# toverainc/willow-inference-server

Measured on AMD Instinct MI355X. Metric: realtime_multiple (audio_ms / infer_ms), Whisper large-v2 beam=5, 3.84 s clip, higher is better.
Workload: dtype f16; 1 GPU; whisper-large beam=5 clip=3sec (3840 ms) batch=1/GPU, PCM resident in HBM -> ids on host; parallelism=1 independent replicas (utterance sharding, no data-path collective)

## Files before the change

### include/wis_hip.h

```cpp
#ifndef WIS_HIP_H
#define WIS_HIP_H

#include <stddef.h>
#include <stdint.h>

#ifdef __cplusplus
extern "C" {
#endif

#define WIS_ABI_VERSION 1

#define WIS_OK             0
#define WIS_E_ARG         -1
#define WIS_E_FORMAT      -2
#define WIS_E_NOMEM       -3
#define WIS_E_CHECKSUM    -4
#define WIS_E_HIP         -5
#define WIS_E_STATE       -6
#define WIS_E_UNSUPPORTED -7

#define WIS_SAMPLE_RATE 16000
#define WIS_N_FFT       400
#define WIS_HOP         160
#define WIS_N_MELS      80
// ... 152 lines not shown
                          int B, int R, int H, int T, int chunks);
int wis_op_dec_cross_attn_folded(int device, const float* q_raw, const float* xres, const float* qcs, const float* qb,
                                 const void* kx_f16, const void* vt_f16, void* out_f16, int B, int R, int H, int T, int chunks);

int wis_op_dec_cross_attn_stat(int device, const float* q, const float* q2, const float* stat, const float* qcs, const float* qb,
                               const void* kx_f16, const void* vt_f16, void* out_f16, int B, int R, int H, int T, int chunks,
                               int out_mb, int kv_shared, int no_spin);
int wis_op_dec_self_attn_ex(int device, const float* q, const void* kc_f16, const void* vc_f16, const int32_t* pos, void* out_f16,
                            int M, int H, int ctx, int rpu, int sstride, int rmul, int nb, int out_mb,
                            const int32_t* anc, int w0, int aw, const int32_t* base);
int wis_op_gemv_qkv(int device, const float* x, const float* gamma, const float* beta, const void* W_f16, const float* bias,
                    const int32_t* slot, const int32_t* pos, float* q, void* kc_f16, void* vc_f16, int M, int d, int ctx);
int wis_op_gemv_out_cq(int device, const void* a_f16, const float* x0, const void* Wo_f16, const float* bo, const void* Wq_f16, const float* bq,
                       const float* gamma, const float* beta, float* x1, float* stat, float* q, float* q2, float* qcs, float* qb,
                       int M, int d, int force_frag);

typedef struct wis_sv wis_sv_t;
typedef struct {
  int32_t conv_dim;
  int32_t n_conv_layers;
  int32_t conv_kernel[8], conv_stride[8];
  int32_t hidden_size, n_heads, n_layers, intermediate_size;
  int32_t num_conv_pos_embeddings, num_conv_pos_embedding_groups;
  int32_t num_buckets, max_bucket_distance;
  int32_t n_tdnn;
  int32_t tdnn_dim[8], tdnn_kernel[8], tdnn_dilation[8];
  int32_t xvector_output_dim;
  int64_t max_samples;
} wis_sv_config_t;
int    wis_sv_create(const wis_sv_config_t* cfg, const void* arena, size_t arena_bytes, int arena_on_device,
// ... 21 lines not shown
```

### willow-inference-server_amd/csrc/dec_kernels.hip

```cpp
#include <string.h>
#include "common.hpp"
#include "kernels.hpp"

namespace wis {

__global__ void pack_gemv_kernel(const f16* __restrict__ W, f16* __restrict__ Wp, int N, int Npad, int K, int n_scale, float scale, int rows) {
  const int ksteps = K / 32;
  const size_t total = (size_t)Npad * ksteps * 4;
  for (size_t idx = (size_t)blockIdx.x * blockDim.x + threadIdx.x; idx < total; idx += (size_t)gridDim.x * blockDim.x) {
    const int row = (int)(idx % rows);
    size_t t = idx / rows;
    const int kq = (int)(t & 3); t >>= 2;
    const int ks = (int)(t % ksteps), nt = (int)(t / ksteps);
    const int n = rows * nt + row, k = 32 * ks + 8 * kq;
    f16x8 v;
    if (n < N) {
      v = *reinterpret_cast<const f16x8*>(W + (size_t)n * K + k);
      if (n < n_scale) {
#pragma unroll
        for (int j = 0; j < 8; ++j) v[j] = (f16)((float)v[j] * scale);
      }
    } else {
#pragma unroll
      for (int j = 0; j < 8; ++j) v[j] = (f16)0.f;
// ... 421 lines not shown
#define WIS_GV_LEAD_DECL(s) const void* s##x, const void* s##x2, const f16* s##Wp, int s##M, int s##N, int s##K, int s##xsplit
#define WIS_GV_LEAD_APPLY(q, s) (q).x = s##x; (q).x2 = s##x2; (q).Wp = s##Wp; (q).M = s##M; (q).N = s##N; (q).K = s##K; (q).xsplit = s##xsplit
template <int MB, int MODE, int SC, int RM, bool W8, int NT = 1>
__global__ __launch_bounds__(256) void gemv_kernel(WIS_GV_LEAD_DECL(l_), int KC, GemvP p) {
  extern __shared__ __attribute__((aligned(16))) char smem[];
  WIS_GV_LEAD_APPLY(p, l_);
  gemv_body<MB, MODE, SC, RM, W8, NT>(p, KC, blockIdx.x, smem);
}
template <int SCA, int SCB>
__global__ __launch_bounds__(256) void gemv_dual_kernel(int nA, int M, const void* ax, const f16* aWp, const void* bx, const void* bx2, const f16* bWp, int bxsplit,
                                                        GemvP pa, GemvP pb) {
  extern __shared__ __attribute__((aligned(16))) char smem[];
  if ((int)blockIdx.x < nA) { pa.x = ax; pa.x2 = nullptr; pa.Wp = aWp; pa.M = M; pa.K = SCA * 128; gemv_body<1, 2, SCA, 1, false>(pa, SCA * 128, blockIdx.x, smem); }
  else { pb.x = bx; pb.x2 = bx2; pb.Wp = bWp; pb.M = M; pb.K = SCB * 128; pb.xsplit = bxsplit; gemv_body<1, 2, SCB, 1, false>(pb, SCB * 128, (int)blockIdx.x - nA, smem); }
}
int launch_gemv_dual(hipStream_t st, const GemvP& pa, const GemvP& pb) {
  if (pa.M != pb.M || pa.M < 1 || pa.M > 16 || pa.x2 || pa.wscale || pb.wscale || (pa.flags & (GV_LN | GV_QKV)) || (pb.flags & (GV_LN | GV_QKV))) { set_error("gemv_dual: unsupported pair"); return WIS_E_UNSUPPORTED; }
  if (pa.M * (pa.K / 8) > 13 * 256 || pb.M * (pb.K / 8) > 13 * 256 || pa.K % 128 || pb.K % 128) { set_error("gemv_dual: rows do not fit the register staging (M=%d K=%d/%d)", pa.M, pa.K, pb.K); return WIS_E_UNSUPPORTED; }
  const int sa = pa.K / 128, sb = pb.K / 128;
  const size_t aux = (size_t)4 * 64 * 16 + MAX_ROWS * 8 + 4 * 16 * 4 + 16;
  const int Kmax = pa.K > pb.K ? pa.K : pb.K;
  const size_t lds = (((size_t)pa.M * (Kmax + 8) * 2 + 15) & ~(size_t)15) + aux;
  if (lds > 65536) { set_error("gemv_dual: LDS"); return WIS_E_UNSUPPORTED; }
  const int nA = cdiv(pa.N, 16), nB = cdiv(pb.N, 16);
  dim3 grid(nA + nB), block(256);
  GemvP a = pa, b = pb; a.rows = 16; b.rows = 16;
  if (sa == 10 && sb == 20) hipLaunchKernelGGL((gemv_dual_kernel<10, 20>), grid, block, lds, st, nA, a.M, a.x, a.Wp, b.x, b.x2, b.Wp, b.xsplit, a, b);
  else if (sa == 8 && sb == 16) hipLaunchKernelGGL((gemv_dual_kernel<8, 16>), grid, block, lds, st, nA, a.M, a.x, a.Wp, b.x, b.x2, b.Wp, b.xsplit, a, b);
  else if (sa == 6 && sb == 12) hipLaunchKernelGGL((gemv_dual_kernel<6, 12>), grid, block, lds, st, nA, a.M, a.x, a.Wp, b.x, b.x2, b.Wp, b.xsplit, a, b);
  else if (sa == 4 && sb == 8) hipLaunchKernelGGL((gemv_dual_kernel<4, 8>), grid, block, lds, st, nA, a.M, a.x, a.Wp, b.x, b.x2, b.Wp, b.xsplit, a, b);
  else if (sa == 3 && sb == 6) hipLaunchKernelGGL((gemv_dual_kernel<3, 6>), grid, block, lds, st, nA, a.M, a.x, a.Wp, b.x, b.x2, b.Wp, b.xsplit, a, b);
  else { set_error("gemv_dual: K=%d/%d not instantiated", pa.K, pb.K); return WIS_E_UNSUPPORTED; }
  return WIS_OK;
// ... 543 lines not shown
  const int m = blockIdx.x;
  const f16* e = emb + (size_t)tok[m] * d;
  const f16* pe = pos_emb + (size_t)pos[m] * d;
  for (int i = threadIdx.x; i < d; i += blockDim.x) {
    const float v = (float)e[i] + (float)pe[i];
    x[(size_t)m * d + i] = v;
    if (xh) xh[(size_t)m * d + i] = (f16)v;
  }
}
int launch_dec_embed(hipStream_t st, const f16* emb, const f16* pos_emb, const int* tok, const int* pos, float* x, int M, int d, f16* xh) {
  hipLaunchKernelGGL(dec_embed_kernel, dim3(M), dim3(256), 0, st, emb, pos_emb, tok, pos, x, xh, d);
  return WIS_OK;
}

template <bool TREE, int NB>
__global__ __launch_bounds__(64) void dec_self_attn_kernel(const float* __restrict__ q, const f16* __restrict__ kc, const f16* __restrict__ vc,
                                                           const int* __restrict__ pos, int d, int ctx, int rpu, int sstride, int rmul,
                                                           f16* __restrict__ out, unsigned long long* prof, int out_mb,
                                                           const int* __restrict__ anc, int w0, int aw, const int* __restrict__ base) {
  __shared__ float red[4][64];
  const int m = blockIdx.x, h = blockIdx.y, lane = threadIdx.x, pl = lane >> 3, c = lane & 7;
  unsigned long long* pf = (m == 0 && h == 0 && lane == 0) ? prof : nullptr;
  if (lane == 0) tl_begin(prof);
  stamp(pf, 0);
  const int ls = TREE ? (base ? base[m] : anc[(size_t)m * aw]) : (m / rpu) * sstride + (m % rpu) * rmul;
  const int len = pos[m] + 1;
  auto slot_of = [&](int p) -> int {
    if (!TREE) return ls;
    int t = p - w0; t = t < aw - 1 ? t : aw - 1;
    return t < 0 ? ls : anc[(size_t)m * aw + t];
  };
  const float4 q0 = *reinterpret_cast<const float4*>(q + (size_t)m * d + h * 64 + 8 * c);
  const float4 q1 = *reinterpret_cast<const float4*>(q + (size_t)m * d + h * 64 + 8 * c + 4);
  const float qv[8] = {q0.x, q0.y, q0.z, q0.w, q1.x, q1.y, q1.z, q1.w};
// ... 72 lines not shown
  } while (p0 < len);
  stamp(pf, 2);
#pragma unroll
  for (int j = 0; j < 8; ++j) acc[j] += dpp_f<0x128>(acc[j]);
  if ((lane & 8) == 0) {
#pragma unroll
    for (int j = 0; j < 8; ++j) red[lane >> 4][8 * c + j] = acc[j];
  }
  __syncthreads();
  stamp(pf, 3);
  const float o = (red[0][lane] + red[1][lane]) + (red[2][lane] + red[3][lane]);
  out[out_mb ? xf_index(m, h * 64 + lane, out_mb) : (size_t)m * d + h * 64 + lane] = (f16)(o / l_run);
  stamp(pf, 4);
  if (lane == 0) tl_end(prof);
}
int launch_dec_self_attn(hipStream_t st, const SelfAttnP& p) {
  if (p.ctx > 512 || p.ctx < 64) { set_error("dec_self_attn: ctx=%d outside [64, 512]", p.ctx); return WIS_E_UNSUPPORTED; }
#define WIS_SA(TREEv, NBv) hipLaunchKernelGGL((dec_self_attn_kernel<TREEv, NBv>), dim3(p.M, p.H), dim3(64), 0, st, p.q, p.kc, p.vc, p.pos, p.d, p.ctx, p.rpu, p.sstride, p.rmul, p.out, \
                                              p.prof, p.out_mb, p.anc, p.w0, p.aw, p.base)
  if (p.anc) {
    if (p.aw < 1) { set_error("dec_self_attn: ancestor table of width %d", p.aw); return WIS_E_ARG; }
    WIS_SA(true, 8);
  } else if (p.nb == 2) WIS_SA(false, 2);
  else if (p.nb == 4) WIS_SA(false, 4);
  else WIS_SA(false, 8);
#undef WIS_SA
  return WIS_OK;
}

__device__ __forceinline__ void st_sc1(float* p, float v) {
  __hip_atomic_store(reinterpret_cast<unsigned*>(p), __float_as_uint(v), __ATOMIC_RELAXED, __HIP_MEMORY_SCOPE_AGENT);
}
// ... 1246 lines not shown
```

### willow-inference-server_amd/csrc/kernels.hpp

```cpp
#pragma once
#include "common.hpp"

namespace wis {

struct GemmP {
  const f16* A; int64_t a_bs; int a_rs; int a_rpb;
  const f16* W;
  int M, N, K;
  int klen;
  int n_span = 0, n_period = 0, n_phase = 0;
};
static inline GemmP gemm_plain(const f16* A, int lda, const f16* W, int M, int N, int K) {
  GemmP p; p.A = A; p.a_bs = 0; p.a_rs = lda; p.a_rpb = 0x7fffffff; p.W = W; p.M = M; p.N = N; p.K = K; p.klen = 0; return p;
}
int launch_layernorm(hipStream_t st, const float* x, const float* gamma, const float* beta, f16* y, int M, int d);
int launch_gemm_generic(hipStream_t st, const GemmP& p, const float* bias, const float* resid, void* C, int flags);
int launch_gemm_splitk_resid(hipStream_t st, const GemmP& p, int splits, float* scratch, const float* bias, const float* resid, float* X,
                             const float* ln_gamma = nullptr, const float* ln_beta = nullptr, f16* Y = nullptr);
int launch_gemm_conv1(hipStream_t st, const GemmP& p, const float* bias, f16* C, int T);
int launch_gemm_conv2(hipStream_t st, const GemmP& p, const float* bias, const float* pos, float* X, int T);
int launch_gemm_qkv(hipStream_t st, const GemmP& p, const float* bias, f16* qk, f16* vt, int d, int T, int Tpad, int H);
int launch_gemm_crosskv(hipStream_t st, const GemmP& p, const float* bias, f16* kx, f16* vt, int d, int T, int Tpad, int H, int64_t kx_lstride, int64_t vt_lstride);
int launch_enc_attention(hipStream_t st, const f16* qk, const f16* vt, f16* out, int B, int T, int Tpad, int H, float* part = nullptr, unsigned* counters = nullptr,
                         size_t part_cap = 0);
// ... 26 lines not shown
  float* q; f16* kc; f16* vc; const int* slot; const int* pos; int d; int ctx;
  unsigned long long* prof;
  int rows;
  const void* x2; int xsplit;
  f16* y16;
  int xmb;
  const float* stat_in;
  float* stat_out;
  f16* y_xf;
  int ymb;
  int ksplit; float* kpart; unsigned* kcnt;
  int mb0, mbi;
  int wks, wk0;
};
int launch_gemv(hipStream_t st, const GemvP& p);
int launch_gemv_dual(hipStream_t st, const GemvP& pa, const GemvP& pb);
int launch_gemv_frag(hipStream_t st, const GemvP& p);
int launch_gemv_frag3(hipStream_t st, const GemvP* p, int n);
__host__ __device__ static inline size_t xf_index(int m, int k, int MB) {
  return ((size_t)((k >> 5) * MB + (m >> 4)) * 64 + (m & 15) + 16 * ((k >> 3) & 3)) * 8 + (k & 7);
}
int launch_xf_pack(hipStream_t st, const void* x, int x_f16, f16* xf, float* stat, int M, int K, int MB);
int launch_dec_embed_xf(hipStream_t st, const f16* emb, const f16* pos_emb, const int* tok, const int* pos, float* x, f16* xf, float* stat, int M, int d, int MB);
int launch_fold_ln(hipStream_t st, f16* W, const float* gamma, const float* beta, float* bias, float* csum, int N, int K, int n_scale, float qscale);
int launch_csum8(hipStream_t st, const f16* W, const float* scale, float* csum, int N, int K, int n_scale, float qscale);
int launch_pack_gemv8(hipStream_t st, const f16* W, unsigned char* Wp, float* scale, int N, int Npad, int K, int n_scale, float qscale);
int launch_pack_gemv(hipStream_t st, const f16* W, f16* Wp, int N, int Npad, int K, int n_scale, float scale, int rows = 16);
int gemv_rows_for(int N, int K);

int launch_dec_embed(hipStream_t st, const f16* emb, const f16* pos_emb, const int* tok, const int* pos, float* x, int M, int d, f16* xh = nullptr);
struct SelfAttnP {
  const float* q = nullptr; const f16* kc = nullptr; const f16* vc = nullptr; const int* pos = nullptr; f16* out = nullptr;
  int M = 0, H = 0, d = 0, ctx = 0, rpu = 0, sstride = 0, rmul = 0;
  unsigned long long* prof = nullptr; int out_mb = 0; const int* anc = nullptr; int w0 = 0, aw = 0;
  const int* base = nullptr;
  int nb = 8;
};
int launch_dec_self_attn(hipStream_t st, const SelfAttnP& p);
constexpr int CA_SPIN_MAX_BH = 192;
struct CrossAttnP {
  const float* q = nullptr; const f16* kx = nullptr; const f16* vt = nullptr; f16* out = nullptr; float* part = nullptr; unsigned* counters = nullptr;
  int B = 0, R = 0, H = 0, d = 0, T = 0, Tpad = 0, chunks = 0;
  unsigned long long* prof = nullptr; int out_mb = 0;
  const float* xres = nullptr; const float* qcs = nullptr; const float* qb = nullptr;
  unsigned long long* gran = nullptr; unsigned* epoch = nullptr;
  const float* q2 = nullptr; int xres_is_stat = 0;
  int kv_shared = 0;
};
int launch_dec_cross_attn(hipStream_t st, const CrossAttnP& p);

struct SampleCfg {
// ... 57 lines not shown
```

### willow-inference-server_amd/csrc/model.hip

```cpp
#include <math.h>
#include <stdlib.h>
#include <string.h>
#include <time.h>
#include <algorithm>
#include <array>
#include <atomic>
#include <chrono>
#include <map>
#include <mutex>
#include <memory>
#include <string>
#include <vector>

#include "common.hpp"
#include "kernels.hpp"

using namespace wis;

namespace wis {

__global__ void convert_kernel(const void* __restrict__ src, int src_f16, void* __restrict__ dst, int dst_f16,
                               int64_t rows, int64_t cols, int64_t dst_ld, int64_t n_scale, float scale) {
  const int64_t total = rows * cols;
  for (int64_t i = (int64_t)blockIdx.x * blockDim.x + threadIdx.x; i < total; i += (int64_t)gridDim.x * blockDim.x) {
// ... 143 lines not shown
  std::vector<DecLayerW> dec;
  f16 *emb, *dec_pos; float *dec_ln_g, *dec_ln_b;
  DecProj proj;
  float *bias_all, *bias_begin; int* d_lang_ids;
  int n_vocab_pad;
  int Tpad;
  f16 *img, *c1, *xn, *qk, *vt, *ao, *hbuf, *mem;
  float* x; float* skbuf; float* enc_part = nullptr; unsigned* enc_cnt = nullptr;
  std::vector<f16*> kx, vx;
  std::vector<f16*> kc, vc;
  f16 *kc_all = nullptr, *vc_all = nullptr; size_t kv_layer_stride = 0;
  f16 *kx_all = nullptr, *vx_all = nullptr, *w_ckv_all = nullptr; float* b_ckv_all = nullptr;
  size_t kx_lstride = 0, vx_lstride = 0;
  float *dx, *dq, *logits, *part; f16 *dao, *dh, *dln; unsigned* counters;
  float* dq2 = nullptr;
  int sa_nb = 8;
  float* gf_part = nullptr; unsigned* gf_cnt = nullptr; int gf_ksplit = 1;
  unsigned long long* ca_gran = nullptr; unsigned* ca_epoch = nullptr;
  bool spin_off = false;
  int handoff_retries = 0;
  bool spin_now = true;
  f16 *dxf = nullptr, *daoxf = nullptr, *dhxf = nullptr; float* dstat = nullptr;
  RowMeta rm; BeamState bs;
  RowMeta rm_win;
  float *st_max, *st_sum, *st_val; int* st_idx;
  int* ts_desc = nullptr;
  float* d_nsp = nullptr;
  int nsp_B = 0;
  float* d_in; int64_t* d_nsamp; float* d_probs;
  int* vstep = nullptr; int* pick_tok = nullptr; float* pick_lp = nullptr;
// ... 277 lines not shown
  WIS_RET(dalloc(m, &m->kc_all, m->kv_layer_stride * L));
  WIS_RET(dalloc(m, &m->vc_all, m->kv_layer_stride * L));
  m->kx_lstride = (size_t)Bm * H * 8 * T * 8; m->vx_lstride = (size_t)Bm * H * 64 * m->Tpad;
  WIS_RET(dalloc(m, &m->kx_all, m->kx_lstride * L));
  WIS_RET(dalloc(m, &m->vx_all, m->vx_lstride * L));
  WIS_HIP_CHECK(hipMemsetAsync(m->vx_all, 0, m->vx_lstride * L * 2, m->st));
  for (int l = 0; l < L; ++l) {
    m->kx[l] = m->kx_all + (size_t)l * m->kx_lstride;
    m->vx[l] = m->vx_all + (size_t)l * m->vx_lstride;
    m->kc[l] = m->kc_all + (size_t)l * slots * ctx * d;
    m->vc[l] = m->vc_all + (size_t)l * slots * ctx * d;
  }
  WIS_RET(dalloc(m, &m->dx, (size_t)MAX_ROWS * d));
  WIS_RET(dalloc(m, &m->dq, (size_t)MAX_ROWS * d));
  WIS_RET(dalloc(m, &m->dq2, (size_t)MAX_ROWS * d));
  WIS_RET(dalloc(m, &m->dao, (size_t)MAX_ROWS * d));
  WIS_RET(dalloc(m, &m->dh, (size_t)MAX_ROWS * 4 * d));
  WIS_RET(dalloc(m, &m->dln, (size_t)MAX_ROWS * d));
  WIS_RET(dalloc(m, &m->dxh, (size_t)MAX_ROWS * d));
  {
    const size_t blk = (size_t)(MAX_ROWS / 16) * 64 * 8;
    WIS_RET(dalloc(m, &m->dxf, (size_t)(d / 32) * blk)); WIS_RET(dalloc(m, &m->daoxf, (size_t)(d / 32) * blk)); WIS_RET(dalloc(m, &m->dhxf, (size_t)(4 * d / 32) * blk));
    WIS_RET(dalloc(m, &m->dstat, (size_t)MAX_ROWS * (d / 16) * 2));
    WIS_HIP_CHECK(hipMemsetAsync(m->dxf, 0, (size_t)(d / 32) * blk * 2, m->st)); WIS_HIP_CHECK(hipMemsetAsync(m->daoxf, 0, (size_t)(d / 32) * blk * 2, m->st));
    WIS_HIP_CHECK(hipMemsetAsync(m->dhxf, 0, (size_t)(4 * d / 32) * blk * 2, m->st));
  }
  WIS_RET(dalloc(m, &m->logits, (size_t)MAX_ROWS * m->n_vocab_pad));
  const int Bg = Bm > MAX_ROWS / 16 ? Bm : MAX_ROWS / 16;
  WIS_RET(dalloc(m, &m->part, (size_t)Bg * H * 16 * 16 * 66));
  WIS_RET(dalloc(m, &m->counters, (size_t)Bg * H));
// ... 176 lines not shown
}

struct TreeWin { const int* anc; int w0, aw; const int* base = nullptr; };
int align_capture_q(wis_model* m, int l, int M);

static GemvP gemv_small(const DecProj& p, const void* x, void* y, int M, int flags) {
  GemvP g; memset(&g, 0, sizeof(g));
  g.x = x; g.csum = p.csum; g.Wp = p.Wp; g.wscale = p.scale; g.bias = p.bias; g.y = y; g.M = M; g.N = p.N; g.K = p.K; g.flags = flags; g.rows = p.rows;
  return g;
}
static GemvP gemv_frag(const DecProj& p, const void* xf, int M, int flags) {
  GemvP g; memset(&g, 0, sizeof(g));
  g.x = xf; g.csum = p.csum; g.Wp = p.Wp; g.wscale = p.scale; g.bias = p.bias; g.M = M; g.N = p.N; g.K = p.K; g.flags = flags; g.xmb = cdiv(M, 16); g.rows = 16;
  return g;
}
static void out_cq_dual(const DecLayerW& w, const f16* a, const f16* xh, float* x1, float* stat, float* q, int M, GemvP* ga, GemvP* gb) {
  const int d = w.out.K;
  memset(ga, 0, sizeof(*ga));
  ga->x = a; ga->Wp = w.out.Wp; ga->bias = w.out.bias; ga->y = x1; ga->M = M; ga->N = d; ga->K = d; ga->flags = GV_RESID; ga->stat_out = stat;
  memset(gb, 0, sizeof(*gb));
  gb->x = xh; gb->x2 = a; gb->xsplit = d; gb->Wp = w.cqo.Wp; gb->bias = w.cqo.bias; gb->y = q; gb->M = M; gb->N = d; gb->K = w.cqo.K; gb->flags = GV_OUT_F32;
}
static void out_cq_frag3(const DecLayerW& w, const f16* af, const f16* xf, float* x1, float* stat, float* q, float* q2, int M, GemvP g3[3]) {
  const int d = w.out.K;
  g3[0] = gemv_frag(w.out, af, M, GV_RESID);
  g3[0].wscale = nullptr; g3[0].y = x1; g3[0].ymb = g3[0].xmb; g3[0].stat_out = stat;
  g3[1] = gemv_frag(w.cqo, xf, M, GV_OUT_F32);
  g3[1].K = d; g3[1].y = q; g3[1].wks = w.cqo.K / 32; g3[1].wk0 = 0;
  g3[2] = gemv_frag(w.cqo, af, M, GV_OUT_F32);
  g3[2].K = d; g3[2].bias = nullptr; g3[2].y = q2; g3[2].wks = w.cqo.K / 32; g3[2].wk0 = d / 32;
}

static int dec_forward_frag(wis_model* m, int M, int R, int B, bool want_logits, int sstride, int rmul, int chunks, const TreeWin* tw = nullptr) {
  const wis_config_t& c = m->cfg; hipStream_t st = m->st;
  const int d = c.d_model, H = c.n_heads, T = c.n_audio_ctx, ctx = c.n_text_ctx, MB = cdiv(M, 16);
  if (tw && (M % 16 != 0 || R != 16 || B != M / 16)) { set_error("dec_forward_frag: a tree window takes whole groups of 16 rows"); return WIS_E_ARG; }
// ... 77 lines not shown
  const int ln = ln16 ? GV_LN16 : GV_LN;
  auto ln_x = [&](const f16* x16) { return ln16 ? (const void*)x16 : (const void*)m->dx; };
  WIS_RET(launch_dec_embed(st, m->emb, m->dec_pos, m->rm.tok, m->rm.pos, m->dx, M, d, fold ? m->dxh : nullptr));
  SelfAttnP sa;
  sa.q = m->dq; sa.pos = m->rm.pos; sa.out = m->dao; sa.M = M; sa.H = H; sa.d = d; sa.ctx = ctx; sa.rpu = R; sa.sstride = sstride; sa.rmul = rmul; sa.nb = m->sa_nb;
  CrossAttnP ca;
  ca.q = m->dq; ca.out = m->dao; ca.part = m->part; ca.counters = m->counters; ca.B = B; ca.R = R; ca.H = H; ca.d = d; ca.T = T; ca.Tpad = m->Tpad; ca.chunks = chunks;
  ca.gran = m->spin_now ? m->ca_gran : nullptr; ca.epoch = m->ca_epoch;
  for (int l = 0; l < c.n_dec_layers; ++l) {
    const DecLayerW& w = m->dec[l];
    unsigned long long* pr = (m->prof_on && (l == 0 || m->prof_all)) ? m->d_prof + (size_t)l * 8 * 16 : nullptr;
    GemvP g = gemv_small(w.qkv, ln_x(m->dxh), nullptr, M, ln | GV_QKV);
    g.q = m->dq; g.kc = m->kc[l]; g.vc = m->vc[l]; g.slot = m->rm.slot; g.pos = m->rm.pos; g.d = d; g.ctx = ctx;
    g.prof = pr;
    WIS_RET(launch_gemv(st, g));
    sa.kc = m->kc[l]; sa.vc = m->vc[l]; sa.prof = pr ? pr + 16 : nullptr;
    WIS_RET(launch_dec_self_attn(st, sa));
    ca.kx = m->kx[l]; ca.vt = m->vx[l]; ca.prof = pr ? pr + 64 : nullptr;
    if (fold) {
      GemvP ga, gb;
      out_cq_dual(w, m->dao, m->dxh, m->dx, m->dstat, m->dq, M, &ga, &gb);
      ga.prof = pr ? pr + 32 : nullptr;
      WIS_RET(launch_gemv_dual(st, ga, gb));
      CrossAttnP cf = ca;
      cf.xres = m->dstat; cf.qcs = w.cq.csum; cf.qb = w.cq.bias; cf.xres_is_stat = 1;
      WIS_RET(launch_dec_cross_attn(st, cf));
    } else {
    g = gemv_small(w.out, m->dao, m->dx, M, GV_RESID);
    g.prof = pr ? pr + 32 : nullptr;
    WIS_RET(launch_gemv(st, g));
    g = gemv_small(w.cq, m->dx, m->dq, M, GV_LN | GV_OUT_F32);
    g.prof = pr ? pr + 48 : nullptr;
    WIS_RET(launch_gemv(st, g));
    WIS_RET(launch_dec_cross_attn(st, ca));
    }
    g = gemv_small(w.cout, m->dao, m->dx, M, GV_RESID);
    g.prof = pr ? pr + 80 : nullptr;
    if (ln16) g.y16 = m->dln;
// ... 323 lines not shown
```

### willow-inference-server_amd/csrc/taps.hip

```cpp
extern "C" {

int wis_debug_encode(wis_model_t* m, const float* input, int input_kind, int B, float* enc_out) {
  if (!m || !input || !enc_out) { set_error("wis_debug_encode: bad argument"); return WIS_E_ARG; }
  WIS_ENTER(m, "wis_debug_encode")
  WIS_HIP_CHECK(hipSetDevice(m->device));
  WIS_RET(check_batch(m, B, 1));
  WIS_RET(stage_input(m, input, input_kind, B));
  WIS_RET(run_encoder(m, B));
  const int64_t n = (int64_t)B * m->cfg.n_audio_ctx * m->cfg.d_model;
  hipLaunchKernelGGL(f16_to_f32_kernel, dim3(blocks_for(n)), dim3(256), 0, m->st, m->mem, m->x, n);
  WIS_HIP_CHECK(hipMemcpyAsync(enc_out, m->x, (size_t)n * 4, hipMemcpyDeviceToHost, m->st));
  WIS_HIP_CHECK(hipStreamSynchronize(m->st));
  return WIS_OK;
}

int wis_debug_logits(wis_model_t* m, const float* input, int input_kind, int B, const int32_t* dec_in, int T, float* logits) {
  if (!m || !input || !dec_in || !logits || T < 1 || T > m->cfg.n_text_ctx) { set_error("wis_debug_logits: bad argument"); return WIS_E_ARG; }
  WIS_ENTER(m, "wis_debug_logits")
  WIS_HIP_CHECK(hipSetDevice(m->device));
  WIS_RET(check_batch(m, B, 1));
  WIS_RET(stage_input(m, input, input_kind, B));
  WIS_RET(run_encoder(m, B));
  WIS_RET(run_cross_kv(m, B));
  const int V = m->cfg.n_vocab;
// ... 469 lines not shown
    else {
      hipMemsetAsync(xf, 0, (size_t)(d / 32) * MB * 64 * 8 * 2, st);
      if ((rc = launch_xf_pack(st, x, 0, xf, stt, M, d, MB))) break;
      g = gemv_frag(qkv, xf, M, GV_LN | GV_QKV);
      g.stat_in = stt;
    }
    g.q = q; g.kc = reinterpret_cast<f16*>(kc); g.vc = reinterpret_cast<f16*>(vc); g.slot = slot; g.pos = pos; g.d = d; g.ctx = ctx;
    rc = M <= 8 ? launch_gemv(st, g) : launch_gemv_frag(st, g);
  } while (0);
  hipError_t e = hipStreamSynchronize(st);
  if (rc) return rc;
  if (e != hipSuccess) { set_error("wis_op_gemv_qkv: %s", hipGetErrorString(e)); return WIS_E_HIP; }
  return WIS_OK;
}

int wis_op_gemv_out_cq(int device, const void* a, const float* x0, const void* Wo, const float* bo, const void* Wq, const float* bq, const float* gamma, const float* beta,
                       float* x1, float* stat, float* q, float* q2, float* qcs, float* qb, int M, int d, int force_frag) {
  DeviceCtx* c; WIS_RET(get_ctx(device, &c));
  std::lock_guard<std::mutex> op_lock(ctx_op_mutex(c));
  const bool frag = M > 8 || force_frag;
  if (!a || !x0 || !Wo || !bo || !Wq || !bq || !gamma || !beta || !x1 || !stat || !q || !qcs || !qb || (frag && !q2) || M < 1 || M > MAX_ROWS || d < 128 || d % 128) {
    set_error("wis_op_gemv_out_cq: bad argument"); return WIS_E_ARG; }
  hipStream_t st = ctx_stream(c);
  const int MB = cdiv(M, 16);
  const float qs = 0.125f;
  const size_t img = (size_t)(d / 32) * MB * 64 * 8;
  TapScratch ts;
  f16 *wtmp = nullptr, *fcat = nullptr, *fwot = nullptr, *fwqo = nullptr, *p_cqo = nullptr, *p_out = nullptr, *xh = nullptr, *xf = nullptr, *af = nullptr; float* b_cqo = nullptr;
  if (!ts.get(&wtmp, (size_t)d * d) || !ts.get(&fcat, (size_t)2 * d * d) || !ts.get(&fwot, (size_t)d * d) || !ts.get(&fwqo, (size_t)d * d) || !ts.get(&p_cqo, (size_t)2 * d * d) ||
      !ts.get(&p_out, (size_t)d * d) || !ts.get(&b_cqo, (size_t)d) || (frag ? (!ts.get(&xf, img) || !ts.get(&af, img)) : !ts.get(&xh, (size_t)M * d))) {
    set_error("wis_op_gemv_out_cq: out of device memory"); return WIS_E_NOMEM; }
  int rc = WIS_OK;
  do {
    hipMemcpyAsync(wtmp, Wq, (size_t)d * d * 2, hipMemcpyDeviceToDevice, st);
    hipLaunchKernelGGL(convert_kernel, dim3(blocks_for(d)), dim3(256), 0, st, bq, 0, qb, 0, (int64_t)d, (int64_t)1, (int64_t)1, (int64_t)d, qs);
    hipMemsetAsync(qcs, 0, (size_t)d * 4, st);
    DecLayerW w{};
    w.out = DecProj{p_out, nullptr, bo, nullptr, d, d, gemv_rows_for(d, d)};
    w.cqo = DecProj{p_cqo, nullptr, b_cqo, nullptr, d, 2 * d, 16};
    if ((rc = prep_projection(st, wtmp, d, d, d, d, qs, gamma, beta, qb, qcs, nullptr, nullptr, 16))) break;
    if ((rc = launch_pack_gemv(st, reinterpret_cast<const f16*>(Wo), p_out, d, d, d, 0, 1.f, w.out.rows))) break;
    if ((rc = build_cq_fold(st, wtmp, Wo, 1, bo, d, qs, fcat, fwot, fwqo, p_cqo, b_cqo))) break;
    hipMemcpyAsync(x1, x0, (size_t)M * d * 4, hipMemcpyDeviceToDevice, st);
    if (!frag) {
      hipLaunchKernelGGL(convert_kernel, dim3(blocks_for((int64_t)M * d)), dim3(256), 0, st, x0, 0, xh, 1, (int64_t)M, (int64_t)d, (int64_t)d, (int64_t)0, 1.f);
      GemvP ga, gb;
      out_cq_dual(w, reinterpret_cast<const f16*>(a), xh, x1, stat, q, M, &ga, &gb);
      rc = launch_gemv_dual(st, ga, gb);
      break;
    }
    hipMemsetAsync(xf, 0, img * 2, st); hipMemsetAsync(af, 0, img * 2, st);
    if ((rc = launch_xf_pack(st, x0, 0, xf, nullptr, M, d, MB))) break;
    if ((rc = launch_xf_pack(st, a, 1, af, nullptr, M, d, MB))) break;
    GemvP g3[3];
    out_cq_frag3(w, af, xf, x1, stat, q, q2, M, g3);
    rc = launch_gemv_frag3(st, g3, 3);
  } while (0);
  hipError_t e = hipStreamSynchronize(st);
  if (rc) return rc;
  if (e != hipSuccess) { set_error("wis_op_gemv_out_cq: %s", hipGetErrorString(e)); return WIS_E_HIP; }
  return WIS_OK;
}

}
```

### willow-inference-server_amd/wis_hip/_lib.py

```python
import ctypes as C
import os

import numpy as np

_HERE = os.path.dirname(os.path.abspath(__file__))
LIB_PATH = os.environ.get("WIS_LIB_PATH") or os.path.join(os.path.dirname(_HERE), "lib", "libwis_hip.so")

WIS_OK = 0
WIS_IN_MEL_HOST, WIS_IN_MEL_DEV, WIS_IN_PCM_HOST, WIS_IN_PCM_DEV = 0, 1, 2, 3
WIS_DT_F32, WIS_DT_F16 = 0, 1
N_SAMPLES, N_FRAMES, N_MELS = 480000, 3000, 80


class WisError(RuntimeError):
    def __init__(self, code, msg):
        super().__init__(f"libwis_hip error {code}: {msg}")
        self.code = code


class Config(C.Structure):
    _fields_ = [(n, C.c_int32) for n in ("d_model", "n_heads", "n_enc_layers", "n_dec_layers", "n_vocab", "n_audio_ctx",
                                          "n_text_ctx", "n_mels", "max_batch", "max_beam", "eot", "sot", "no_timestamps",
                                          "no_speech")] + [
        ("suppress_ids", C.POINTER(C.c_int32)), ("n_suppress", C.c_int32),
# ... 82 lines not shown
    ("wis_dev_h2d", _i, [_i, _vp, _vp, _sz]),
    ("wis_dev_d2h", _i, [_i, _vp, _vp, _sz]),
    ("wis_dev_sync", _i, [_i]),
    ("wis_dev_copy_peer", _i, [_i, _vp, _i, _vp, _sz]),
    ("wis_op_gemm", _i, [_i, _vp, _i, _vp, _vp, _vp, _vp, _i, _i, _i, _i]),
    ("wis_op_layernorm", _i, [_i, _vp, _vp, _vp, _vp, _i, _i]),
    ("wis_op_enc_attention", _i, [_i, _vp, _vp, _vp, _i, _i, _i, _i]),
    ("wis_op_gemv", _i, [_i, _vp, _vp, _vp, _vp, _vp, _vp, _i, _i, _i, _i]),
    ("wis_op_dec_self_attn", _i, [_i, _vp, _vp, _vp, _vp, _vp, _i, _i, _i, _i, _i, _i]),
    ("wis_op_dec_cross_attn", _i, [_i, _vp, _vp, _vp, _vp, _i, _i, _i, _i, _i]),
    ("wis_op_dec_cross_attn_folded", _i, [_i, _vp, _vp, _vp, _vp, _vp, _vp, _vp, _i, _i, _i, _i, _i]),
    ("wis_op_dec_cross_attn_stat", _i, [_i] + [_vp] * 8 + [_i] * 8),
    ("wis_op_dec_self_attn_ex", _i, [_i, _vp, _vp, _vp, _vp, _vp, _i, _i, _i, _i, _i, _i, _i, _i, _vp, _i, _i, _vp]),
    ("wis_op_gemv_qkv", _i, [_i] + [_vp] * 10 + [_i] * 3),
    ("wis_op_gemv_out_cq", _i, [_i] + [_vp] * 14 + [_i] * 3),
    ("wis_sv_create", _i, [C.POINTER(SvConfig), _vp, _sz, _i, C.POINTER(Tensor), _i, _i, C.POINTER(_vp)]),
    ("wis_sv_destroy", None, [_vp]),
    ("wis_sv_device_bytes", _sz, [_vp]),
    ("wis_sv_embed", _i, [_vp, _vp, _i64, _fp]),
    ("wis_sv_rel_buckets", _i, [_i, _i, _i, _i, C.POINTER(C.c_int32)]),
    ("wis_debug_sv_taps", _i, [_vp, _vp, _i64, _i, _i, _fp, _i64, C.POINTER(C.c_int32), C.POINTER(C.c_int32)]),
    ("wis_op_sv_conv0", _i, [_i, _vp, _i64, _vp, _vp, _vp, _vp]),
    ("wis_op_sv_posconv", _i, [_i, _vp, _vp, _vp, _vp, _i]),
    ("wis_op_sv_attention", _i, [_i, _vp, _vp, _vp, _vp, _vp, _vp, _i, _vp, _i]),
    ("wis_op_sv_layernorm", _i, [_i, _vp, _i, _vp, _vp, _vp, _vp, _vp, _vp, C.c_float, _i, _i, _i]),
    ("wis_op_sv_xvector_tail", _i, [_i, _vp, _i, _i, _i, _vp, _vp, _vp, _vp]),
]

_lib = None

# ... 72 lines not shown
```

Measured before the change: 148.1 x realtime.

## Compute residual half of folded cross-Q projection inside self-attention launch

The folded cross-attention Q projection has two halves, one over the pre-attention residual and one over the attention output. The half that only needs the residual is now computed by extra blocks added to the self-attention kernel's grid, writing partial sums to a scratch buffer. The later dual gemv then only computes the attention-output half and adds the stored partials plus bias. The aim is to use idle compute units during the latency-bound self-attention step and shorten the critical-path gemv, at the cost of an extra partial-sum buffer round trip and more kernel complexity; it can be turned off with WIS_CQ_EARLY=0.

After: 149.1 x realtime, median of 6. No clear change (+0.7%).

```diff
diff --git a/include/wis_hip.h b/include/wis_hip.h
--- a/include/wis_hip.h
+++ b/include/wis_hip.h
@@ -190,6 +190,8 @@
 int wis_op_gemv_out_cq(int device, const void* a_f16, const float* x0, const void* Wo_f16, const float* bo, const void* Wq_f16, const float* bq,
                        const float* gamma, const float* beta, float* x1, float* stat, float* q, float* q2, float* qcs, float* qb,
                        int M, int d, int force_frag);
+int wis_op_out_cq_early(int device, const void* a_f16, const float* x0, const void* Wo_f16, const float* bo, const void* Wq_f16, const float* bq,
+                        const float* gamma, const float* beta, float* x1, float* stat, float* q, int M, int d, int early);
 
 typedef struct wis_sv wis_sv_t;
 typedef struct {
diff --git a/willow-inference-server_amd/csrc/dec_kernels.hip b/willow-inference-server_amd/csrc/dec_kernels.hip
--- a/willow-inference-server_amd/csrc/dec_kernels.hip
+++ b/willow-inference-server_amd/csrc/dec_kernels.hip
@@ -459,9 +459,116 @@
   if ((int)blockIdx.x < nA) { pa.x = ax; pa.x2 = nullptr; pa.Wp = aWp; pa.M = M; pa.K = SCA * 128; gemv_body<1, 2, SCA, 1, false>(pa, SCA * 128, blockIdx.x, smem); }
   else { pb.x = bx; pb.x2 = bx2; pb.Wp = bWp; pb.M = M; pb.K = SCB * 128; pb.xsplit = bxsplit; gemv_body<1, 2, SCB, 1, false>(pb, SCB * 128, (int)blockIdx.x - nA, smem); }
 }
-int launch_gemv_dual(hipStream_t st, const GemvP& pa, const GemvP& pb) {
+template <int S>
+__device__ __forceinline__ void cq_first_wave(const f16* __restrict__ x, const f16* __restrict__ Wp, const int M, const int unit, float* __restrict__ P, char* smem) {
+  constexpr int d = 64 * S, c8 = 4 * S, xstr = 32 * S + 8;
+  constexpr int NXH = 8 * c8 / 64;
+  const int lane = threadIdx.x, nt = unit >> 1, kw = unit & 1;
+  f16* xs = reinterpret_cast<f16*>(smem);
+  const int nx = M * c8;
+  u32x4 xh[NXH];
+  const u32x4* x8 = reinterpret_cast<const u32x4*>(x) + kw * c8;
+#pragma unroll
+  for (int i = 0; i < NXH; ++i) { const int idx = lane + 64 * i; if (idx < nx) { const int row = idx / c8; xh[i] = x8[(size_t)row * (d / 8) + (idx - row * c8)]; } }
+  u32x4 wf[S];
+  const u32x4* wq = reinterpret_cast<const u32x4*>(Wp) + ((size_t)nt * (4 * S) + kw * S) * 64 + lane;
+#pragma unroll
+  for (int u = 0; u < S; ++u) wf[u] = __builtin_nontemporal_load(wq + (size_t)u * 64);
+#pragma unroll
+  for (int i = 0; i < NXH; ++i) {
+    const int idx = lane + 64 * i;
+    if (idx < nx) { const int row = idx / c8, k8 = idx - row * c8; *reinterpret_cast<u32x4*>(xs + (size_t)row * xstr + k8 * 8) = xh[i]; }
+  }
+  __syncthreads();
+  const int ep_m = lane & 15, ep_n = 16 * nt + 4 * (lane >> 4);
+  const int xrow = (ep_m < M ? ep_m : M - 1) * xstr + 8 * (lane >> 4);
+  f32x4 acc = f32x4{0.f, 0.f, 0.f, 0.f};
+#pragma unroll
+  for (int u = 0; u < S; ++u) {
+    const f16x8 xb = *reinterpret_cast<const f16x8*>(xs + xrow + u * 32);
+    acc = __builtin_amdgcn_mfma_f32_16x16x32_f16(*reinterpret_cast<const f16x8*>(&wf[u]), xb, acc, 0, 0, 0);
+  }
+  if (ep_m < M) *reinterpret_cast<float4*>(P + ((size_t)kw * M + ep_m) * d + ep_n) = make_float4(acc[0], acc[1], acc[2], acc[3]);
+}
+template <int S>
+__device__ __forceinline__ void cq_second_body(const f16* __restrict__ x, const f16* __restrict__ Wp, const int M, const int nt, const float* __restrict__ P,
+                                               const float* __restrict__ bias, float* __restrict__ y, char* smem) {
+  constexpr int d = 64 * S, c8 = d / 8, xstr = d + 8;
+  constexpr int NXH = (8 * c8 + 255) / 256;
+  const int tid = threadIdx.x, lane = tid & 63, wave = __builtin_amdgcn_readfirstlane(tid >> 6);
+  f16* xs = reinterpret_cast<f16*>(smem);
+  float* red = reinterpret_cast<float*>(smem + (((size_t)M * xstr * 2 + 15) & ~(size_t)15));
+  const int nx = M * c8;
+  u32x4 xh[NXH];
+  const u32x4* x8 = reinterpret_cast<const u32x4*>(x);
+#pragma unroll
+  for (int i = 0; i < NXH; ++i) { const int idx = tid + 256 * i; if (idx < nx) xh[i] = x8[idx]; }
+  u32x4 wf[S];
+  if (wave < 2) {
+    const u32x4* wq = reinterpret_cast<const u32x4*>(Wp) + ((size_t)nt * (4 * S) + (2 + wave) * S) * 64 + lane;
+#pragma unroll
+    for (int u = 0; u < S; ++u) wf[u] = __builtin_nontemporal_load(wq + (size_t)u * 64);
+  }
+#pragma unroll
+  for (int i = 0; i < NXH; ++i) {
+    const int idx = tid + 256 * i;
+    if (idx < nx) { const int row = idx / c8, k8 = idx - row * c8; *reinterpret_cast<u32x4*>(xs + (size_t)row * xstr + k8 * 8) = xh[i]; }
+  }
+  __syncthreads();
+  f32x4 acc = f32x4{0.f, 0.f, 0.f, 0.f};
+  const int ep_m = lane & 15, ep_n = 16 * nt + 4 * (lane >> 4);
+  const bool ep_ok = wave == 0 && ep_m < M;
+  float4 ep_bias = make_float4(0.f, 0.f, 0.f, 0.f), ep_t0 = ep_bias, ep_t1 = ep_bias;
+  if (wave < 2) {
+    const int xrow = (ep_m < M ? ep_m : M - 1) * xstr + 8 * (lane >> 4);
+#pragma unroll
+    for (int u = 0; u < S; ++u) {
+      const f16x8 xb = *reinterpret_cast<const f16x8*>(xs + xrow + (wave * S + u) * 32);
+      acc = __builtin_amdgcn_mfma_f32_16x16x32_f16(*reinterpret_cast<const f16x8*>(&wf[u]), xb, acc, 0, 0, 0);
+    }
+    if (ep_ok) {
+      ep_bias = *reinterpret_cast<const float4*>(bias + ep_n);
+      ep_t0 = *reinterpret_cast<const float4*>(P + (size_t)ep_m * d + ep_n);
+      ep_t1 = *reinterpret_cast<const float4*>(P + ((size_t)M + ep_m) * d + ep_n);
+    }
+    if (wave == 1) *reinterpret_cast<float4*>(red + (size_t)lane * 4) = make_float4(acc[0], acc[1], acc[2], acc[3]);
+  }
+  __syncthreads();
+  if (ep_ok) {
+    const float4 t3 = *reinterpret_cast<const float4*>(red + (size_t)lane * 4);
+    float4 s = make_float4(0.f, 0.f, 0.f, 0.f);
+    s.x += ep_t0.x; s.y += ep_t0.y; s.z += ep_t0.z; s.w += ep_t0.w;
+    s.x += ep_t1.x; s.y += ep_t1.y; s.z += ep_t1.z; s.w += ep_t1.w;
+    s.x += acc[0]; s.y += acc[1]; s.z += acc[2]; s.w += acc[3];
+    s.x += t3.x; s.y += t3.y; s.z += t3.z; s.w += t3.w;
+    s.x += ep_bias.x; s.y += ep_bias.y; s.z += ep_bias.z; s.w += ep_bias.w;
+    *reinterpret_cast<float4*>(y + (size_t)ep_m * d + ep_n) = s;
+  }
+}
+template <int SCA, int SCB>
+__global__ __launch_bounds__(256) void gemv_dual_early_kernel(int nA, int M, const void* ax, const f16* aWp, const f16* bWp, const float* bP, const float* bbias, float* by,
+                                                              GemvP pa) {
+  extern __shared__ __attribute__((aligned(16))) char smem[];
+  static_assert(SCB == 2 * SCA, "the folded cross-Q's halves are as wide as the out-projection");
+  if ((int)blockIdx.x < nA) { pa.x = ax; pa.x2 = nullptr; pa.Wp = aWp; pa.M = M; pa.K = SCA * 128; gemv_body<1, 2, SCA, 1, false>(pa, SCA * 128, blockIdx.x, smem); }
+  else cq_second_body<SCB>(reinterpret_cast<const f16*>(ax), bWp, M, (int)blockIdx.x - nA, bP, bbias, by, smem);
+}
+int launch_gemv_dual(hipStream_t st, const GemvP& pa, const GemvP& pb, const float* P) {
   if (pa.M != pb.M || pa.M < 1 || pa.M > 16 || pa.x2 || pa.wscale || pb.wscale || (pa.flags & (GV_LN | GV_QKV)) || (pb.flags & (GV_LN | GV_QKV))) { set_error("gemv_dual: unsupported pair"); return WIS_E_UNSUPPORTED; }
   if (pa.M * (pa.K / 8) > 13 * 256 || pb.M * (pb.K / 8) > 13 * 256 || pa.K % 128 || pb.K % 128) { set_error("gemv_dual: rows do not fit the register staging (M=%d K=%d/%d)", pa.M, pa.K, pb.K); return WIS_E_UNSUPPORTED; }
+  if (P) {
+    if (pb.x != pa.x || pb.x2 || pb.K != pa.K || pb.N != pb.K || pb.wks != 2 * (pb.K / 32) || pb.wk0 != pb.K / 32 || pb.flags != GV_OUT_F32 || !pb.bias || pa.M > 8) {
+      set_error("gemv_dual: not the second half of a folded cross-Q (M=%d K=%d/%d)", pa.M, pa.K, pb.K); return WIS_E_UNSUPPORTED; }
+    const size_t lds = (((size_t)pa.M * (pa.K + 8) * 2 + 15) & ~(size_t)15) + (size_t)4 * 64 * 16 + MAX_ROWS * 8 + 4 * 16 * 4 + 16;
+    const int nA = cdiv(pa.N, 16);
+    dim3 grid(nA + pb.N / 16), block(256);
+    GemvP a = pa; a.rows = 16;
+#define WIS_DE(SCAv) hipLaunchKernelGGL((gemv_dual_early_kernel<SCAv, 2 * SCAv>), grid, block, lds, st, nA, a.M, a.x, a.Wp, pb.Wp, P, pb.bias, reinterpret_cast<float*>(pb.y), a)
+    switch (pa.K / 128) { case 10: WIS_DE(10); break; case 8: WIS_DE(8); break; case 6: WIS_DE(6); break; case 4: WIS_DE(4); break; case 3: WIS_DE(3); break;
+      default: set_error("gemv_dual: K=%d not instantiated", pa.K); return WIS_E_UNSUPPORTED; }
+#undef WIS_DE
+    return WIS_OK;
+  }
   const int sa = pa.K / 128, sb = pb.K / 128;
   const size_t aux = (size_t)4 * 64 * 16 + MAX_ROWS * 8 + 4 * 16 * 4 + 16;
   const int Kmax = pa.K > pb.K ? pa.K : pb.K;
@@ -1035,10 +1142,10 @@
 }
 
 template <bool TREE, int NB>
-__global__ __launch_bounds__(64) void dec_self_attn_kernel(const float* __restrict__ q, const f16* __restrict__ kc, const f16* __restrict__ vc,
-                                                           const int* __restrict__ pos, int d, int ctx, int rpu, int sstride, int rmul,
-                                                           f16* __restrict__ out, unsigned long long* prof, int out_mb,
-                                                           const int* __restrict__ anc, int w0, int aw, const int* __restrict__ base) {
+__device__ __forceinline__ void dec_self_attn_body(const float* __restrict__ q, const f16* __restrict__ kc, const f16* __restrict__ vc,
+                                                   const int* __restrict__ pos, const int d, int ctx, int rpu, int sstride, int rmul,
+                                                   f16* __restrict__ out, unsigned long long* prof, int out_mb,
+                                                   const int* __restrict__ anc, int w0, int aw, const int* __restrict__ base) {
   __shared__ float red[4][64];
   const int m = blockIdx.x, h = blockIdx.y, lane = threadIdx.x, pl = lane >> 3, c = lane & 7;
   unsigned long long* pf = (m == 0 && h == 0 && lane == 0) ? prof : nullptr;
@@ -1141,8 +1248,44 @@
   stamp(pf, 4);
   if (lane == 0) tl_end(prof);
 }
+template <bool TREE, int NB>
+__global__ __launch_bounds__(64) void dec_self_attn_kernel(const float* __restrict__ q, const f16* __restrict__ kc, const f16* __restrict__ vc,
+                                                           const int* __restrict__ pos, int d, int ctx, int rpu, int sstride, int rmul,
+                                                           f16* __restrict__ out, unsigned long long* prof, int out_mb,
+                                                           const int* __restrict__ anc, int w0, int aw, const int* __restrict__ base) {
+  dec_self_attn_body<TREE, NB>(q, kc, vc, pos, d, ctx, rpu, sstride, rmul, out, prof, out_mb, anc, w0, aw, base);
+}
+template <int NB, int S>
+__global__ __launch_bounds__(64) void dec_self_attn_cqp_kernel(const f16* __restrict__ px, const f16* __restrict__ pWp, const float* __restrict__ q,
+                                                               const f16* __restrict__ kc, const f16* __restrict__ vc, const int* __restrict__ pos,
+                                                               int shape, int smap,
+                                                               f16* __restrict__ out, float* __restrict__ pP, unsigned long long* prof) {
+  extern __shared__ __attribute__((aligned(16))) char smem[];
+  if ((int)blockIdx.y >= S) {
+    const int M = shape >> 24, unit = ((int)blockIdx.y - S) * M + (int)blockIdx.x;
+    if (unit < 8 * S) cq_first_wave<S>(px, pWp, M, unit, pP, smem);
+    return;
+  }
+  dec_self_attn_body<false, NB>(q, kc, vc, pos, 64 * S, shape & 0xFFFF, (shape >> 16) & 0xFF, smap & 0xFFFF, smap >> 16, out, prof, 0, nullptr, 0, 0, nullptr);
+}
 int launch_dec_self_attn(hipStream_t st, const SelfAttnP& p) {
   if (p.ctx > 512 || p.ctx < 64) { set_error("dec_self_attn: ctx=%d outside [64, 512]", p.ctx); return WIS_E_UNSUPPORTED; }
+  if (p.ride) {
+    const GemvP& r = *p.ride;
+    const int S = p.d / 64;
+    if (p.anc || p.out_mb || p.d != 64 * p.H || p.M < 1 || p.M > 8 || p.rpu < 1 || p.rpu > 0xFF || p.sstride < 0 || p.sstride > 0xFFFF || p.rmul < 0 || p.rmul > 0x7FFF || r.M != p.M || r.K != p.d || r.N != p.d || r.wks != 2 * (p.d / 32) || r.wk0 != 0 ||
+        r.x2 || r.bias || r.wscale || r.flags != GV_OUT_F32 || !r.x || !r.Wp || !r.y) { set_error("dec_self_attn: the riding problem is not the first half of a folded cross-Q (M=%d d=%d)", p.M, p.d); return WIS_E_UNSUPPORTED; }
+    const size_t lds = (size_t)p.M * (p.d / 2 + 8) * 2;
+    const dim3 grid(p.M, p.H + cdiv(8 * S, p.M)), block(64);
+#define WIS_SAP(NBv, Sv) hipLaunchKernelGGL((dec_self_attn_cqp_kernel<NBv, Sv>), grid, block, lds, st, reinterpret_cast<const f16*>(r.x), r.Wp, p.q, p.kc, p.vc, p.pos, p.ctx | (p.rpu << 16) | (p.M << 24), \
+                                            p.sstride | (p.rmul << 16), p.out, reinterpret_cast<float*>(r.y), p.prof)
+#define WIS_SAP_NB(Sv) do { if (p.nb == 2) WIS_SAP(2, Sv); else if (p.nb == 4) WIS_SAP(4, Sv); else WIS_SAP(8, Sv); } while (0)
+    switch (S) { case 20: WIS_SAP_NB(20); break; case 16: WIS_SAP_NB(16); break; case 12: WIS_SAP_NB(12); break; case 8: WIS_SAP_NB(8); break; case 6: WIS_SAP_NB(6); break;
+      default: set_error("dec_self_attn: d=%d has no instantiation with the riding cross-Q half", p.d); return WIS_E_UNSUPPORTED; }
+#undef WIS_SAP_NB
+#undef WIS_SAP
+    return WIS_OK;
+  }
 #define WIS_SA(TREEv, NBv) hipLaunchKernelGGL((dec_self_attn_kernel<TREEv, NBv>), dim3(p.M, p.H), dim3(64), 0, st, p.q, p.kc, p.vc, p.pos, p.d, p.ctx, p.rpu, p.sstride, p.rmul, p.out, \
                                               p.prof, p.out_mb, p.anc, p.w0, p.aw, p.base)
   if (p.anc) {
diff --git a/willow-inference-server_amd/csrc/kernels.hpp b/willow-inference-server_amd/csrc/kernels.hpp
--- a/willow-inference-server_amd/csrc/kernels.hpp
+++ b/willow-inference-server_amd/csrc/kernels.hpp
@@ -64,7 +64,7 @@
   int wks, wk0;
 };
 int launch_gemv(hipStream_t st, const GemvP& p);
-int launch_gemv_dual(hipStream_t st, const GemvP& pa, const GemvP& pb);
+int launch_gemv_dual(hipStream_t st, const GemvP& pa, const GemvP& pb, const float* P = nullptr);
 int launch_gemv_frag(hipStream_t st, const GemvP& p);
 int launch_gemv_frag3(hipStream_t st, const GemvP* p, int n);
 __host__ __device__ static inline size_t xf_index(int m, int k, int MB) {
@@ -85,6 +85,7 @@
   unsigned long long* prof = nullptr; int out_mb = 0; const int* anc = nullptr; int w0 = 0, aw = 0;
   const int* base = nullptr;
   int nb = 8;
+  const GemvP* ride = nullptr;
 };
 int launch_dec_self_attn(hipStream_t st, const SelfAttnP& p);
 constexpr int CA_SPIN_MAX_BH = 192;
diff --git a/willow-inference-server_amd/csrc/model.hip b/willow-inference-server_amd/csrc/model.hip
--- a/willow-inference-server_amd/csrc/model.hip
+++ b/willow-inference-server_amd/csrc/model.hip
@@ -181,6 +181,7 @@
   size_t kx_lstride = 0, vx_lstride = 0;
   float *dx, *dq, *logits, *part; f16 *dao, *dh, *dln; unsigned* counters;
   float* dq2 = nullptr;
+  float* dqp = nullptr;
   int sa_nb = 8;
   float* gf_part = nullptr; unsigned* gf_cnt = nullptr; int gf_ksplit = 1;
   unsigned long long* ca_gran = nullptr; unsigned* ca_epoch = nullptr;
@@ -488,6 +489,7 @@
   WIS_RET(dalloc(m, &m->dx, (size_t)MAX_ROWS * d));
   WIS_RET(dalloc(m, &m->dq, (size_t)MAX_ROWS * d));
   WIS_RET(dalloc(m, &m->dq2, (size_t)MAX_ROWS * d));
+  WIS_RET(dalloc(m, &m->dqp, (size_t)2 * MAX_R * d));
   WIS_RET(dalloc(m, &m->dao, (size_t)MAX_ROWS * d));
   WIS_RET(dalloc(m, &m->dh, (size_t)MAX_ROWS * 4 * d));
   WIS_RET(dalloc(m, &m->dln, (size_t)MAX_ROWS * d));
@@ -694,12 +696,22 @@
   g.x = xf; g.csum = p.csum; g.Wp = p.Wp; g.wscale = p.scale; g.bias = p.bias; g.M = M; g.N = p.N; g.K = p.K; g.flags = flags; g.xmb = cdiv(M, 16); g.rows = 16;
   return g;
 }
-static void out_cq_dual(const DecLayerW& w, const f16* a, const f16* xh, float* x1, float* stat, float* q, int M, GemvP* ga, GemvP* gb) {
+static void out_cq_dual(const DecLayerW& w, const f16* a, const f16* xh, float* x1, float* stat, float* q, float* P, int M, GemvP* ga, GemvP* gb, GemvP* gp) {
   const int d = w.out.K;
   memset(ga, 0, sizeof(*ga));
   ga->x = a; ga->Wp = w.out.Wp; ga->bias = w.out.bias; ga->y = x1; ga->M = M; ga->N = d; ga->K = d; ga->flags = GV_RESID; ga->stat_out = stat;
   memset(gb, 0, sizeof(*gb));
+  memset(gp, 0, sizeof(*gp));
+  if (P) {
+    gp->x = xh; gp->Wp = w.cqo.Wp; gp->y = P; gp->M = M; gp->N = d; gp->K = d; gp->flags = GV_OUT_F32; gp->wks = w.cqo.K / 32; gp->wk0 = 0;
+    gb->x = a; gb->Wp = w.cqo.Wp; gb->bias = w.cqo.bias; gb->y = q; gb->M = M; gb->N = d; gb->K = d; gb->flags = GV_OUT_F32; gb->wks = w.cqo.K / 32; gb->wk0 = d / 32;
+    return;
+  }
   gb->x = xh; gb->x2 = a; gb->xsplit = d; gb->Wp = w.cqo.Wp; gb->bias = w.cqo.bias; gb->y = q; gb->M = M; gb->N = d; gb->K = w.cqo.K; gb->flags = GV_OUT_F32;
+}
+static bool cq_early() {
+  static const bool on = !(getenv("WIS_CQ_EARLY") && atoi(getenv("WIS_CQ_EARLY")) == 0);
+  return on;
 }
 static void out_cq_frag3(const DecLayerW& w, const f16* af, const f16* xf, float* x1, float* stat, float* q, float* q2, int M, GemvP g3[3]) {
   const int d = w.out.K;
@@ -807,14 +819,15 @@
     g.q = m->dq; g.kc = m->kc[l]; g.vc = m->vc[l]; g.slot = m->rm.slot; g.pos = m->rm.pos; g.d = d; g.ctx = ctx;
     g.prof = pr;
     WIS_RET(launch_gemv(st, g));
-    sa.kc = m->kc[l]; sa.vc = m->vc[l]; sa.prof = pr ? pr + 16 : nullptr;
+    GemvP ga, gb, gp;
+    float* const P = fold && cq_early() ? m->dqp : nullptr;
+    if (fold) out_cq_dual(w, m->dao, m->dxh, m->dx, m->dstat, m->dq, P, M, &ga, &gb, &gp);
+    sa.kc = m->kc[l]; sa.vc = m->vc[l]; sa.prof = pr ? pr + 16 : nullptr; sa.ride = P ? &gp : nullptr;
     WIS_RET(launch_dec_self_attn(st, sa));
     ca.kx = m->kx[l]; ca.vt = m->vx[l]; ca.prof = pr ? pr + 64 : nullptr;
     if (fold) {
-      GemvP ga, gb;
-      out_cq_dual(w, m->dao, m->dxh, m->dx, m->dstat, m->dq, M, &ga, &gb);
       ga.prof = pr ? pr + 32 : nullptr;
-      WIS_RET(launch_gemv_dual(st, ga, gb));
+      WIS_RET(launch_gemv_dual(st, ga, gb, P));
       CrossAttnP cf = ca;
       cf.xres = m->dstat; cf.qcs = w.cq.csum; cf.qb = w.cq.bias; cf.xres_is_stat = 1;
       WIS_RET(launch_dec_cross_attn(st, cf));
diff --git a/willow-inference-server_amd/csrc/taps.hip b/willow-inference-server_amd/csrc/taps.hip
--- a/willow-inference-server_amd/csrc/taps.hip
+++ b/willow-inference-server_amd/csrc/taps.hip
@@ -507,8 +507,10 @@
   return WIS_OK;
 }
 
-int wis_op_gemv_out_cq(int device, const void* a, const float* x0, const void* Wo, const float* bo, const void* Wq, const float* bq, const float* gamma, const float* beta,
-                       float* x1, float* stat, float* q, float* q2, float* qcs, float* qb, int M, int d, int force_frag) {
+}
+
+static int op_out_cq(int device, const void* a, const float* x0, const void* Wo, const float* bo, const void* Wq, const float* bq, const float* gamma, const float* beta,
+                     float* x1, float* stat, float* q, float* q2, float* qcs, float* qb, int M, int d, int force_frag, bool early) {
   DeviceCtx* c; WIS_RET(get_ctx(device, &c));
   std::lock_guard<std::mutex> op_lock(ctx_op_mutex(c));
   const bool frag = M > 8 || force_frag;
@@ -537,9 +539,22 @@
     hipMemcpyAsync(x1, x0, (size_t)M * d * 4, hipMemcpyDeviceToDevice, st);
     if (!frag) {
       hipLaunchKernelGGL(convert_kernel, dim3(blocks_for((int64_t)M * d)), dim3(256), 0, st, x0, 0, xh, 1, (int64_t)M, (int64_t)d, (int64_t)d, (int64_t)0, 1.f);
-      GemvP ga, gb;
-      out_cq_dual(w, reinterpret_cast<const f16*>(a), xh, x1, stat, q, M, &ga, &gb);
-      rc = launch_gemv_dual(st, ga, gb);
+      GemvP ga, gb, gp;
+      float* P = nullptr;
+      if (early && !ts.get(&P, (size_t)2 * M * d)) { set_error("wis_op_gemv_out_cq: out of device memory"); rc = WIS_E_NOMEM; break; }
+      out_cq_dual(w, reinterpret_cast<const f16*>(a), xh, x1, stat, q, P, M, &ga, &gb, &gp);
+      if (early) {
+        const int H = d / 64, sctx = 64;
+        float* sq = nullptr; f16 *skv = nullptr, *so = nullptr; int* spos = nullptr;
+        if (!ts.get(&sq, (size_t)M * d) || !ts.get(&skv, (size_t)M * sctx * d) || !ts.get(&so, (size_t)M * d) || !ts.get(&spos, (size_t)M)) {
+          set_error("wis_op_gemv_out_cq: out of device memory"); rc = WIS_E_NOMEM; break; }
+        hipMemsetAsync(sq, 0, (size_t)M * d * 4, st); hipMemsetAsync(skv, 0, (size_t)M * sctx * d * 2, st); hipMemsetAsync(spos, 0, (size_t)M * 4, st);
+        hipMemsetAsync(P, 0xFF, (size_t)2 * M * d * 4, st);
+        SelfAttnP sa;
+        sa.q = sq; sa.kc = skv; sa.vc = skv; sa.pos = spos; sa.out = so; sa.M = M; sa.H = H; sa.d = d; sa.ctx = sctx; sa.rpu = M; sa.sstride = M; sa.rmul = 1; sa.nb = 2; sa.ride = &gp;
+        if ((rc = launch_dec_self_attn(st, sa))) break;
+      }
+      rc = launch_gemv_dual(st, ga, gb, P);
       break;
     }
     hipMemsetAsync(xf, 0, img * 2, st); hipMemsetAsync(af, 0, img * 2, st);
@@ -555,4 +570,20 @@
   return WIS_OK;
 }
 
-}
+extern "C" {
+
+int wis_op_gemv_out_cq(int device, const void* a, const float* x0, const void* Wo, const float* bo, const void* Wq, const float* bq, const float* gamma, const float* beta,
+                       float* x1, float* stat, float* q, float* q2, float* qcs, float* qb, int M, int d, int force_frag) {
+  return op_out_cq(device, a, x0, Wo, bo, Wq, bq, gamma, beta, x1, stat, q, q2, qcs, qb, M, d, force_frag, cq_early());
+}
+int wis_op_out_cq_early(int device, const void* a, const float* x0, const void* Wo, const float* bo, const void* Wq, const float* bq, const float* gamma, const float* beta,
+                        float* x1, float* stat, float* q, int M, int d, int early) {
+  if (M > 8 || d < 128 || d % 128) { set_error("wis_op_out_cq_early: the one-utterance stage takes at most 8 rows (M=%d d=%d)", M, d); return WIS_E_ARG; }
+  float *qcs = nullptr, *qb = nullptr;
+  TapScratch ts;
+  { DeviceCtx* c; WIS_RET(get_ctx(device, &c)); }
+  if (!ts.get(&qcs, (size_t)d) || !ts.get(&qb, (size_t)d)) { set_error("wis_op_out_cq_early: out of device memory"); return WIS_E_NOMEM; }
+  return op_out_cq(device, a, x0, Wo, bo, Wq, bq, gamma, beta, x1, stat, q, nullptr, qcs, qb, M, d, 0, early != 0);
+}
+
+}
diff --git a/willow-inference-server_amd/wis_hip/_lib.py b/willow-inference-server_amd/wis_hip/_lib.py
--- a/willow-inference-server_amd/wis_hip/_lib.py
+++ b/willow-inference-server_amd/wis_hip/_lib.py
@@ -120,6 +120,7 @@
     ("wis_op_dec_self_attn_ex", _i, [_i, _vp, _vp, _vp, _vp, _vp, _i, _i, _i, _i, _i, _i, _i, _i, _vp, _i, _i, _vp]),
     ("wis_op_gemv_qkv", _i, [_i] + [_vp] * 10 + [_i] * 3),
     ("wis_op_gemv_out_cq", _i, [_i] + [_vp] * 14 + [_i] * 3),
+    ("wis_op_out_cq_early", _i, [_i] + [_vp] * 11 + [_i] * 3),
     ("wis_sv_create", _i, [C.POINTER(SvConfig), _vp, _sz, _i, C.POINTER(Tensor), _i, _i, C.POINTER(_vp)]),
     ("wis_sv_destroy", None, [_vp]),
     ("wis_sv_device_bytes", _sz, [_vp]),
```
